# arnavsshah/universal-voice-activity-detection

Hardware: AMD Instinct MI355X
Metric: audio frames/sec (log-mel + PyanNet2 VAD forward); per-frame logit max-abs-err vs CPU ref (higher is better)
Workload: dtype f16x4: f32-equivalent arithmetic on the f16 matrix cores -- exact f32 weights as 3 f16 planes x activations as 2 f16 planes (22 bits), 4 matrix products per f32 product (v_mfma_f32_*_f16; in the recurrence the fourth -- the weights' residue plane, exactly representable as bf8, times h rounded to fp8

## Files before the change

universal-voice-activity-detection_amd/csrc/gemm_f16p_ws.hip:

```cpp
#include "uvad_internal.h"

#include <type_traits>
#include <utility>

namespace uvad {

namespace {

using f32x16 = __attribute__((ext_vector_type(16))) float;
using f16x8 = __attribute__((ext_vector_type(8))) _Float16;
using f32x4 = __attribute__((ext_vector_type(4))) float;
typedef const __attribute__((address_space(1))) void *gptr_t;
typedef __attribute__((address_space(3))) void *lptr_t;

constexpr int SLAB = 128 * 16;
constexpr int STAGE = 2 * SLAB;
constexpr int GROUPS = 8;

template <class F, int... I> __device__ __forceinline__ void static_for_impl(F &&f, std::integer_sequence<int, I...>) {
    (f(std::integral_constant<int, I>{}), ...);
}
template <int N, class F> __device__ __forceinline__ void static_for(F &&f) { static_for_impl(f, std::make_integer_sequence<int, N>{}); }

template <int NKB> struct Ring { static constexpr int NST = NKB % 8 == 0 ? 8 : NKB % 6 == 0 ? 6 : 4; };

template <int N> __device__ __forceinline__ void wait_vm() {
    static_assert(N >= 0 && N <= 63, "vmcnt is a 6-bit counter");
    __builtin_amdgcn_s_waitcnt(0x0f70 | (N & 0xf) | ((N >> 4) << 14));
}

constexpr int NPIECE = 16;
template <int NKB> constexpr int piece_begin(int kb) { return kb >= NKB - 1 ? NPIECE : kb <= 0 ? 0 : (NPIECE * kb) / (NKB - 1); }
template <int NKB> constexpr int stores_in(int from, int to) {
    int n = 0;
    for (int j = from < 1 ? 1 : from; j < to; ++j) n += piece_begin<NKB>(j) - piece_begin<NKB>(j - 1);
    return n;
}

template <int N> __device__ __forceinline__ void wait_vm_lgkm0() {
    static_assert(N >= 0 && N <= 63, "vmcnt is a 6-bit counter");
    __builtin_amdgcn_s_waitcnt(0x0070 | (N & 0xf) | ((N >> 4) << 14));
}

template <int NKB, int NPROD>
__global__ __launch_bounds__(256, 1) void gemm_f16p_ws_kernel(GemmArgs a, int mt, int nt, unsigned *counters) {
    constexpr int NST = Ring<NKB>::NST;
    static_assert(NKB % 2 == 0 && NKB % NST == 0 && NST - 1 <= NKB && NST >= 4, "ring / fragment double-buffer geometry");
    constexpr int SG_LD = 36;
    constexpr int SG_WAVE = 128 * SG_LD * 2;
    __shared__ __attribute__((aligned(16))) unsigned short lds[NST * STAGE + 4 * SG_WAVE + 16];
    int *qword = reinterpret_cast<int *>(lds + NST * STAGE + 4 * SG_WAVE);

    if (a.gate && (*a.gate != 0) != (a.gate_run_if_set != 0)) return;
    const int bid = blockIdx.x, grp = bid & (GROUPS - 1);
    const int n_tile = (bid >> 3) % nt;
    const int tid = threadIdx.x, lane = tid & 63;
    const int wave = __builtin_amdgcn_readfirstlane(tid >> 6);
    const int fr = lane & 31, fh = lane >> 5;

    unsigned *ctr = counters + (size_t)(grp * nt + n_tile) * 32;
    typedef const __attribute__((address_space(4))) int *cint_t;
    cint_t lst = nullptr;
    if (a.ws_tiles) {
        const int d = (a.ws_dirs == 2 && n_tile >= nt / 2) ? 1 : 0;
        lst = (cint_t)(unsigned long long)(a.ws_tiles + a.ws_off[d]);
        mt = a.ws_len[d];
    }
    auto rowtile = [&](int c) { const int i = grp + GROUPS * c; return lst ? lst[i] : i; };
    const int my_tiles = mt > grp ? (mt - grp + GROUPS - 1) / GROUPS : 0;
    if (tid == 0) {
        qword[0] = (int)atomicAdd(ctr, 1u);
        qword[1] = (int)atomicAdd(ctr, 1u);
    }
    __syncthreads();
    int c_cur = __builtin_amdgcn_readfirstlane(qword[0]), c_nxt = __builtin_amdgcn_readfirstlane(qword[1]);
    if ((unsigned)c_cur >= (unsigned)my_tiles) return;
    int r_cur = __builtin_amdgcn_readfirstlane(rowtile(c_cur));
    int r_nxt = (unsigned)c_nxt < (unsigned)my_tiles ? __builtin_amdgcn_readfirstlane(rowtile(c_nxt)) : r_cur;

    static_assert(NPROD == 3 || NPROD == 4, "three or four products");
    f16x8 w0[NKB], w1[NKB], w2[NPROD == 4 ? NKB : 1];
    {
        const size_t wplane = (size_t)((a.N + 127) / 128) * NKB * SLAB;
        const unsigned short *wb = a.Wsplit16 + (size_t)n_tile * NKB * SLAB + (wave * 32 + fr) * 16 + fh * 8;
#pragma unroll
        for (int kb = 0; kb < NKB; ++kb) {
            w0[kb] = *reinterpret_cast<const f16x8 *>(wb + (size_t)kb * SLAB);
            w1[kb] = *reinterpret_cast<const f16x8 *>(wb + wplane + (size_t)kb * SLAB);
            if constexpr (NPROD == 4) w2[kb] = *reinterpret_cast<const f16x8 *>(wb + 2 * wplane + (size_t)kb * SLAB);
        }
    }
    float bias[16];
#pragma unroll
    for (int r = 0; r < 16; ++r) bias[r] = a.bias ? a.bias[n_tile * 128 + wave * 32 + 8 * (r >> 2) + 4 * fh + (r & 3)] : 0.f;
    const float wscale = a.wscale;
    const unsigned q_addr = (unsigned)(size_t)(lptr_t)qword;

    const int ra = tid >> 1;
    const unsigned off = (unsigned)((ra * 2 + ((tid & 1) ^ ((ra >> 3) & 1))) * 8);
    const unsigned short *a_hi = a.Ah + off, *a_lo = a.Al + off;
    auto issue = [&](int stage, int rt, int kb) {
        const size_t t = (size_t)rt * NKB + kb;
        unsigned short *img = lds + stage * STAGE + wave * 512;
        __builtin_amdgcn_global_load_lds((gptr_t)(a_hi + t * SLAB), (lptr_t)(img), 16, 0, 0);
        __builtin_amdgcn_global_load_lds((gptr_t)(a_lo + t * SLAB), (lptr_t)(img + SLAB), 16, 0, 0);
    };

    const unsigned f_base = (unsigned)(size_t)(lptr_t)lds + (unsigned)((fr * 16 + ((fh ^ ((fr >> 3) & 1)) * 8)) * 2);
    f16x8 ah[2][4], al[2][4];
#define UVAD_WS_READ(dst, byte_off) asm volatile("ds_read_b128 %0, %1 offset:%2" : "=v"(dst) : "v"(f_base), "n"(byte_off))
#define UVAD_WS_READ_FRAGS(set, stage)                                                                                       \
    {                                                                                                                      \
        constexpr int base_ = (stage) * (STAGE * 2);                                                                       \
        UVAD_WS_READ(ah[set][0], base_ + 0 * 1024); UVAD_WS_READ(ah[set][1], base_ + 1 * 1024);                            \
        UVAD_WS_READ(ah[set][2], base_ + 2 * 1024); UVAD_WS_READ(ah[set][3], base_ + 3 * 1024);                            \
        UVAD_WS_READ(al[set][0], base_ + SLAB * 2 + 0 * 1024); UVAD_WS_READ(al[set][1], base_ + SLAB * 2 + 1 * 1024);      \
        UVAD_WS_READ(al[set][2], base_ + SLAB * 2 + 2 * 1024); UVAD_WS_READ(al[set][3], base_ + SLAB * 2 + 3 * 1024);      \
    }
    static_assert((NST - 1) * STAGE * 2 + SLAB * 2 + 3 * 1024 < 65536, "DS offset field is 16 bits");

#pragma unroll
    for (int v = 0; v < NST - 1; ++v) issue(v, v < NKB ? r_cur : r_nxt, v % NKB);
    wait_vm<2 * (NST - 2)>();
    __builtin_amdgcn_s_barrier();
    UVAD_WS_READ_FRAGS(0, 0)

    f32x16 hi[4], lo[4];
    const f32x16 zero = {0.f, 0.f, 0.f, 0.f, 0.f, 0.f, 0.f, 0.f, 0.f, 0.f, 0.f, 0.f, 0.f, 0.f, 0.f, 0.f};
    float *sg_w = reinterpret_cast<float *>(lds + NST * STAGE + wave * SG_WAVE) + fr * SG_LD + 4 * fh;
    const unsigned sg_r = (unsigned)(size_t)(lptr_t)(lds + NST * STAGE + wave * SG_WAVE) + (unsigned)(((lane >> 3) * SG_LD + (lane & 7) * 4) * 4);
    const size_t g_lane = (size_t)(lane >> 3) * 64 + (wave & 1) * 32 + (lane & 7) * 4;
    const size_t g_ntile = (size_t)n_tile * 2 + (wave >> 1);
    const int n64 = a.N / 64;
    float *gprev = nullptr;
    f32x4 pc[NPIECE];
#define UVAD_WS_READ_PIECE(p) asm volatile("ds_read_b128 %0, %1 offset:%2" : "=v"(pc[p]) : "v"(sg_r), "n"((p) * 8 * SG_LD * 4))
    static_assert(15 * 8 * SG_LD * 4 < 65536, "DS offset field is 16 bits");
    static_assert(piece_begin<NKB>(1) <= 6 && NPIECE - piece_begin<NKB>(NKB - 2) <= 6, "at most six pieces per k-block (UVAD_WS_PIECES)");

    auto tile = [&](auto first_tag) __attribute__((always_inline)) {
        constexpr bool FIRST = decltype(first_tag)::value;
#pragma unroll
        for (int kb = 0; kb < NKB; ++kb) {
            asm volatile("" : "+a"(w0[kb]), "+a"(w1[kb]));
            if constexpr (NPROD == 4) asm volatile("" : "+a"(w2[kb]));
        }
        float *gout = a.C + ((size_t)r_cur * n64 + g_ntile) * (128 * 64) + g_lane;
        unsigned pulled = 0;
        (void)pc; (void)sg_r;
        static_for<NKB>([&](auto kb_tag) __attribute__((always_inline)) {
            constexpr int kb = decltype(kb_tag)::value;
            constexpr int s = kb & 1, sn = (kb + 1) & 1, stn = (kb + 1) % NST;
            constexpr bool LAST = kb == NKB - 1;
            auto M = [&](auto j_tag) __attribute__((always_inline)) {
                constexpr int j = decltype(j_tag)::value, i = j & 3, p = j >> 2;
                if constexpr (p == 0) hi[i] = __builtin_amdgcn_mfma_f32_32x32x16_f16(w0[kb], ah[s][i], kb == 0 ? zero : hi[i], 0, 0, 0);
                if constexpr (p == 1) lo[i] = __builtin_amdgcn_mfma_f32_32x32x16_f16(w1[kb], ah[s][i], kb == 0 ? zero : lo[i], 0, 0, 0);
                if constexpr (p == 2) lo[i] = __builtin_amdgcn_mfma_f32_32x32x16_f16(w0[kb], al[s][i], lo[i], 0, 0, 0);
                if constexpr (p == 3 && NPROD == 4) lo[i] = __builtin_amdgcn_mfma_f32_32x32x16_f16(w2[kb], ah[s][i], lo[i], 0, 0, 0);
            };
            auto stage_block = [&](int i) __attribute__((always_inline)) {
#pragma unroll
                for (int q = 0; q < 4; ++q) {
                    float4 o;
                    o.x = __builtin_fmaf(__builtin_fmaf(lo[i][4 * q + 0], 0.00048828125f, hi[i][4 * q + 0]), wscale, bias[4 * q + 0]);
                    o.y = __builtin_fmaf(__builtin_fmaf(lo[i][4 * q + 1], 0.00048828125f, hi[i][4 * q + 1]), wscale, bias[4 * q + 1]);
                    o.z = __builtin_fmaf(__builtin_fmaf(lo[i][4 * q + 2], 0.00048828125f, hi[i][4 * q + 2]), wscale, bias[4 * q + 2]);
                    o.w = __builtin_fmaf(__builtin_fmaf(lo[i][4 * q + 3], 0.00048828125f, hi[i][4 * q + 3]), wscale, bias[4 * q + 3]);
                    *reinterpret_cast<float4 *>(sg_w + i * (32 * SG_LD) + 8 * q) = o;
                }
            };
#define UVAD_WS_M(j) M(std::integral_constant<int, (j)>{})
#define UVAD_WS_SB __builtin_amdgcn_sched_barrier(0)
#define UVAD_WS_PIECE_IF(kb_, t_) \
    if constexpr (piece_begin<NKB>(kb_) + (t_) < piece_begin<NKB>((kb_) + 1)) UVAD_WS_READ_PIECE(piece_begin<NKB>(kb_) + (t_));
#define UVAD_WS_STORE_IF(t_)                                                                            \
    if constexpr (piece_begin<NKB>(kb - 1) + (t_) < piece_begin<NKB>(kb))                               \
        __builtin_nontemporal_store(pc[piece_begin<NKB>(kb - 1) + (t_)], reinterpret_cast<f32x4 *>(gprev + (size_t)(piece_begin<NKB>(kb - 1) + (t_)) * (8 * 64)));
            UVAD_WS_SB;
            wait_vm_lgkm0<2 * (NST - 3) + (FIRST ? 0 : stores_in<NKB>(kb - (NST - 3), kb))>();
            __builtin_amdgcn_s_barrier();
            UVAD_WS_SB;
            constexpr int v = kb - 1 + NST;
            const int vr = v < NKB ? r_cur : r_nxt;
            const size_t vt = ((size_t)vr * NKB + v % NKB) * SLAB;
            unsigned short *img = lds + ((kb + NST - 1) % NST) * STAGE + wave * 512;
            constexpr int fb = stn * (STAGE * 2);
#define UVAD_WS_GAP(g)                                                                                                           \
    {                                                                                                                            \
        if constexpr (!FIRST && kb >= 1 && (g) == 0) {                             \
            UVAD_WS_STORE_IF(0) UVAD_WS_STORE_IF(1) UVAD_WS_STORE_IF(2) UVAD_WS_STORE_IF(3) UVAD_WS_STORE_IF(4) UVAD_WS_STORE_IF(5)          \
        }                                                                                                                        \
        if constexpr ((g) == 0) __builtin_amdgcn_global_load_lds((gptr_t)(a_hi + vt), (lptr_t)(img), 16, 0, 0);                   \
        if constexpr ((g) == 1) __builtin_amdgcn_global_load_lds((gptr_t)(a_lo + vt), (lptr_t)(img + SLAB), 16, 0, 0);            \
        if constexpr ((g) == 1) { UVAD_WS_READ(ah[sn][0], fb + 0 * 1024); UVAD_WS_READ(ah[sn][1], fb + 1 * 1024); }              \
        if constexpr ((g) == 2) { UVAD_WS_READ(ah[sn][2], fb + 2 * 1024); UVAD_WS_READ(ah[sn][3], fb + 3 * 1024); }              \
        if constexpr ((g) == 3) { UVAD_WS_READ(al[sn][0], fb + SLAB * 2 + 0 * 1024); UVAD_WS_READ(al[sn][1], fb + SLAB * 2 + 1 * 1024); } \
        if constexpr ((g) == 4) { UVAD_WS_READ(al[sn][2], fb + SLAB * 2 + 2 * 1024); UVAD_WS_READ(al[sn][3], fb + SLAB * 2 + 3 * 1024); } \
        if constexpr ((g) == 5 && !FIRST && !LAST) {                 \
            UVAD_WS_PIECE_IF(kb, 0) UVAD_WS_PIECE_IF(kb, 1) UVAD_WS_PIECE_IF(kb, 2) UVAD_WS_PIECE_IF(kb, 3) UVAD_WS_PIECE_IF(kb, 4) UVAD_WS_PIECE_IF(kb, 5) \
        }                                                                                                                        \
        if constexpr (LAST && (g) == 2) stage_block(0);                                                                          \
        if constexpr (LAST && (g) == 4) stage_block(1);                                                                          \
        if constexpr (LAST && (g) == 6) stage_block(2);                                                                          \
        if constexpr (LAST && (g) == 7) stage_block(3);                                                                          \
        UVAD_WS_SB;                                                                                                              \
    }
            if (kb == 0) {
                unsigned long long sv;
                asm volatile("v_cmp_eq_u32_e32 vcc, 0, %2\n\ts_and_saveexec_b64 %1, vcc\n\tglobal_atomic_add %0, %3, %4, off sc0\n\ts_mov_b64 exec, %1"
                             : "=&v"(pulled), "=&s"(sv) : "v"(tid), "v"(ctr), "v"(1u) : "vcc", "memory");
                UVAD_WS_SB;
            }
            if (kb == NST - 2) {
                unsigned long long sv;
                asm volatile("v_cmp_eq_u32_e32 vcc, 0, %1\n\ts_and_saveexec_b64 %0, vcc\n\tds_write_b32 %2, %3\n\ts_waitcnt lgkmcnt(0)\n\ts_mov_b64 exec, %0"
                             : "=&s"(sv) : "v"(tid), "v"(q_addr), "v"(pulled) : "vcc", "memory");
                UVAD_WS_SB;
            }
            if constexpr (!LAST) {
                UVAD_WS_M(0); UVAD_WS_M(1); UVAD_WS_SB; UVAD_WS_GAP(0)
                UVAD_WS_M(2); UVAD_WS_M(3); UVAD_WS_SB; UVAD_WS_GAP(1)
                UVAD_WS_M(4); UVAD_WS_M(5); UVAD_WS_SB; UVAD_WS_GAP(2)
                UVAD_WS_M(6); UVAD_WS_M(7); UVAD_WS_SB; UVAD_WS_GAP(3)
                UVAD_WS_M(8); UVAD_WS_M(9); UVAD_WS_SB; UVAD_WS_GAP(4)
                UVAD_WS_M(10); UVAD_WS_M(11); UVAD_WS_SB; UVAD_WS_GAP(5)
                UVAD_WS_M(12); UVAD_WS_M(13); UVAD_WS_SB; UVAD_WS_GAP(6)
                UVAD_WS_M(14); UVAD_WS_M(15); UVAD_WS_SB; UVAD_WS_GAP(7)
            } else {
                UVAD_WS_M(0); UVAD_WS_M(4); UVAD_WS_SB; UVAD_WS_GAP(0)
                UVAD_WS_M(8); UVAD_WS_M(12); UVAD_WS_SB; UVAD_WS_GAP(1)
                UVAD_WS_M(1); UVAD_WS_M(5); UVAD_WS_SB; UVAD_WS_GAP(2)
                UVAD_WS_M(9); UVAD_WS_M(13); UVAD_WS_SB; UVAD_WS_GAP(3)
                UVAD_WS_M(2); UVAD_WS_M(6); UVAD_WS_SB; UVAD_WS_GAP(4)
                UVAD_WS_M(10); UVAD_WS_M(14); UVAD_WS_SB; UVAD_WS_GAP(5)
                UVAD_WS_M(3); UVAD_WS_M(7); UVAD_WS_SB; UVAD_WS_GAP(6)
                UVAD_WS_M(11); UVAD_WS_M(15); UVAD_WS_SB; UVAD_WS_GAP(7)
            }
        });
        int c_nn;
        asm volatile("ds_read_b32 %0, %1\n\ts_waitcnt lgkmcnt(0)" : "=v"(c_nn) : "v"(q_addr) : "memory");
        gprev = gout;
        c_cur = c_nxt;
        r_cur = r_nxt;
        c_nxt = __builtin_amdgcn_readfirstlane(c_nn);
        r_nxt = (unsigned)c_nxt < (unsigned)my_tiles ? __builtin_amdgcn_readfirstlane(rowtile(c_nxt)) : r_cur;
    };
    tile(std::true_type{});
    for (int done = 1; done < my_tiles && (unsigned)c_cur < (unsigned)my_tiles; ++done) tile(std::false_type{});
    static_for<NPIECE>([&](auto t) __attribute__((always_inline)) {
        constexpr int p = decltype(t)::value;
        f32x4 o;
        asm volatile("ds_read_b128 %0, %1 offset:%2\n\ts_waitcnt lgkmcnt(0)" : "=v"(o) : "v"(sg_r), "n"(p * 8 * SG_LD * 4) : "memory");
        __builtin_nontemporal_store(o, reinterpret_cast<f32x4 *>(gprev + (size_t)p * (8 * 64)));
    });
    wait_vm<0>();
}

}

size_t gemm_f16p_ws_counter_bytes() { return (size_t)GROUPS * 8 * 32 * sizeof(unsigned); }

bool gemm_f16p_ws_supported(const GemmArgs &a, int n_cu) {
    if (a.out_planes || !a.c_blocked || a.act != 0 || a.N % 128 != 0 || a.N / 128 > 8) return false;
    if (a.K != 64 && a.K != 96 && a.K != 128 && a.K != 256) return false;
    const long mt = (a.M + 127) / 128;
    return mt * (a.N / 128) >= 2L * (n_cu > 0 ? n_cu : 256);
}

hipError_t launch_gemm_f16p_ws(const GemmArgs &a, unsigned *counters, int n_cu, hipStream_t s) {
    if (!gemm_f16p_ws_supported(a, n_cu) || !counters || !a.Ah || !a.Al || !a.Wsplit16 || !a.C || a.ldw != a.K) return hipErrorInvalidValue;
    const int mt = (a.M + 127) / 128, nt = a.N / 128;
    if (a.ws_tiles) {
        if ((a.ws_dirs != 1 && a.ws_dirs != 2) || (a.ws_dirs == 2 && nt % 2 != 0)) return hipErrorInvalidValue;
        for (int d = 0; d < a.ws_dirs; ++d)
            if (a.ws_off[d] < 0 || a.ws_len[d] < 0 || a.ws_len[d] > mt) return hipErrorInvalidValue;
    }
    hipError_t e = launch_zero_counters(counters, (int)(gemm_f16p_ws_counter_bytes() / sizeof(unsigned)), s);
    if (e != hipSuccess) return e;
    const int per = GROUPS * nt;
    int grid = (n_cu > 0 ? n_cu : 256) / per * per;
    if (grid < per) grid = per;
    if (a.products != 0 && a.products != 3 && a.products != 4) return hipErrorInvalidValue;
    const bool three = a.products == 3;
#define UVAD_WS_LAUNCH(NKB_)                                                                                                          \
    if (three) hipLaunchKernelGGL((gemm_f16p_ws_kernel<NKB_, 3>), dim3(grid), dim3(256), 0, s, a, mt, nt, counters);                   \
    else hipLaunchKernelGGL((gemm_f16p_ws_kernel<NKB_, 4>), dim3(grid), dim3(256), 0, s, a, mt, nt, counters);
    switch (a.K / 16) {
        case 4: UVAD_WS_LAUNCH(4) break;
        case 6: UVAD_WS_LAUNCH(6) break;
        case 8: UVAD_WS_LAUNCH(8) break;
        case 16: UVAD_WS_LAUNCH(16) break;
        default: return hipErrorInvalidValue;
    }
#undef UVAD_WS_LAUNCH
    return hipGetLastError();
}

}
```

universal-voice-activity-detection_amd/csrc/uvad_internal.h:

```cpp
#pragma once
#include <hip/hip_runtime.h>
#include <type_traits>
#include <stdint.h>

namespace uvad {

constexpr int SEQ_TILE = 4;

constexpr int PLANE_TILE = 128;
__host__ __device__ inline size_t plane_index(size_t row, int col, int width) {
    return ((row / PLANE_TILE) * (size_t)(width / 16) + (size_t)(col / 16)) * (PLANE_TILE * 16) + (row % PLANE_TILE) * 16 + (size_t)(col % 16);
}
inline size_t plane_rows(size_t M) { return (M + PLANE_TILE - 1) / PLANE_TILE * PLANE_TILE; }

__host__ __device__ inline size_t g_index(size_t row, int col, int ncols) {
    return ((row / 128) * (size_t)(ncols / 64) + (size_t)(col / 64)) * (128 * 64) + (row % 128) * 64 + (size_t)(col % 64);
}

struct GemmArgs {
    const float *A;
    const float *W;
    const unsigned short *Ah, *Al;
    const unsigned short *Wsplit16;
    float wscale;
    unsigned short *Ch, *Cl;
    int out_planes;
    int products;
    int c_blocked;
    int ldw;
    const float *bias;
    float *C;
    int M, N, K;
    int lda, ldc;
    int a_mode, B, T;
    float leaky_slope;
    int act;
    const int *gate;
    int gate_run_if_set;
    const int *ws_tiles;
    int ws_off[2], ws_len[2], ws_dirs;
};
hipError_t launch_gemm(const GemmArgs &a, hipStream_t s);
int gemm_padded_k(int K);
hipError_t launch_gemm_f16p(const GemmArgs &a, hipStream_t s);
int gemm_f16p_padded_k(int K);
bool gemm_f16p_ws_supported(const GemmArgs &a, int n_cu);
size_t gemm_f16p_ws_counter_bytes();
hipError_t launch_gemm_f16p_ws(const GemmArgs &a, unsigned *counters, int n_cu, hipStream_t s);
size_t weight_plane_elems(int N, int ldw);
bool split_weights_f16x3(const float *w, int N, int ldw, unsigned short *out , float *wscale);
hipError_t launch_mask_features(const float *x, int B, int T, int F, const int *lens, float *out, hipStream_t s);
hipError_t launch_split_features(const float *x, int B, int T, int F, int Fp, int tiles, unsigned short *xh, unsigned short *xl, int *flag,
                                 hipStream_t s);

struct LstmArgs {
    const float *G; int ldg;
    const float *Whh_packed;
    const unsigned *Whh16h_regs; const unsigned short *Whh16h_p2; const float *whh16h_scale;
    const unsigned short *Whh16h_p2q; int p2q_scale;
    float *Y; int ldy;
    unsigned short *Yh, *Yl;
    int products;
    int tiles, T, H, dirs;
    int steps, t_begin[2];
    int tile_mode;
    int n_cu;
    const float *h0, *c0; float *hN, *cN;
    const int *lens; int nB;
};
hipError_t launch_lstm(const LstmArgs &a, hipStream_t s, int *tile_used = nullptr);
int lstm_auto_tile(int tiles, int dirs, int H, int n_cu);
size_t whh_packed_elems(int H);
int lstm_waves(int H);
void pack_whh(const float *w_hh, int H, float *out);
size_t whh16h_regs_elems();
size_t whh16h_p2_elems();
bool pack_whh16h(const float *w_hh, unsigned *regs, unsigned short *p2, float *wscale);
size_t whh16h_p2q_elems();
bool pack_whh16h_p2q(const float *w_hh, unsigned short *p2q, int *scale);

struct ClsArgs {
    const float *Z; int ldz, K;
    const float *w, *b;
    float *logits, *probs;
    int tiles, T, B;
    int ld_out;
};
hipError_t launch_classifier(const ClsArgs &a, hipStream_t s);
hipError_t launch_untile(const void *src, const void *src_lo, int lds_, int W, float *dst, int tiles, int T, int B, hipStream_t s);
hipError_t launch_median(const float *probs, int B, int T, int kernel, uint8_t *labels, hipStream_t s);
hipError_t launch_runs(const uint8_t *labels, int B, int T, int max_runs, int *runs, int *counts, hipStream_t s);
hipError_t launch_lens_fill(float *logits, float *probs, int B, int T, int ld, const int *lens, hipStream_t s);
hipError_t launch_median_lens(const float *probs, int B, int T, int kernel, uint8_t *labels, const int *lens, hipStream_t s);
hipError_t launch_runs_lens(const uint8_t *labels, int B, int T, int max_runs, int *runs, int *counts, const int *lens, hipStream_t s);
hipError_t launch_der(const uint8_t *pred, const uint8_t *gt, int B, int T, uint32_t *counts, hipStream_t s);

hipError_t launch_zero_counters(unsigned *p, int n, hipStream_t s);

hipError_t launch_spin(unsigned long long ticks, unsigned long long *sink, hipStream_t s);

struct HeadArgs {
    const unsigned short *Yh, *Yl;
    long long M; int K1;
    const unsigned short *W1, *W2;
    float w1scale, w2scale;
    const float *b1, *b2, *wc, *bc;
    float slope;
    float *logits, *probs;
    int tiles, T, B, ld_out;
    unsigned *counter;
    int products;
};
bool head_fused_supported(int K1, int lin_hidden, int lin_layers, long long M, int n_cu);
hipError_t launch_head_fused(const HeadArgs &a, int n_cu, hipStream_t s);

struct FbankTables {
    const float *window;
    const int *mel_start;
    const int *mel_len;
    const float *mel_w;
    const float *mel_wt;
    int mel_stride;
    const float *tw512;
    int nyquist;
};
__host__ __device__ inline int mel_image_ld(int n_mels) { return n_mels <= 64 ? 64 : 128; }
__host__ __device__ inline size_t mel_image_floats(int mel_stride, int n_mels) { return (size_t)mel_stride * mel_image_ld(n_mels); }
struct FbankArgs {
    const void *pcm; int pcm_is_i16;
    int B; int64_t S; int64_t T;
    int64_t row_stride;
    int frame_len, frame_shift, n_mels;
    float preemph, log_floor; int remove_dc, snip_edges;
    float *feats;
    unsigned short *plane_hi, *plane_lo; int plane_w;
    const float *vs_chunk, *vs_tail_in; float *vs_tail_out;
    int vs_tail, vs_chunk_len, vs_first, vs_n_left, vs_offset;
    FbankTables tab;
    const int64_t *nsamp;
};
hipError_t launch_fbank(const FbankArgs &a, hipStream_t s);
hipError_t launch_frames_of(const int64_t *nsamp, int B, int64_t S, int frame_len, int frame_shift, int snip_edges, int *frames, hipStream_t s);
size_t fbank_lds_bytes(const FbankArgs &a);
hipError_t launch_stream_stage(const float *chunk_pcm, int B, int chunk, int tail, int n_left, int first_step,
                               const float *tail_in, float *tail_out, float *staging, hipStream_t s);

struct WindowArgs {
    const float *newf; float *ring; const long long *ctr_in; long long *ctr_out;
    int B, R, F, k, Tw;
    int planes; unsigned short *xh, *xl; int Fp, tiles;
    float *out;
};
hipError_t launch_window_assemble(const WindowArgs &a, hipStream_t s);
hipError_t launch_window_carry(const long long *ctr_in, long long *ctr_out, hipStream_t s);
hipError_t launch_window_emit(const float *logits_in, const float *probs_in, int B, int Tw, int r0, int n, float *logits, float *probs,
                              int ld_out, hipStream_t s);

struct WavWindowArgs {
    const void *chunk; void *ring; const long long *ctr_in; long long *ctr_out;
    int B, chunk_len, J, R, Tw, Sw;
    long long ring_len;
    void *out;
};
hipError_t launch_wav_window_assemble(const WavWindowArgs &a, int is_i16, hipStream_t s);

struct SlotCounters { long long *n, *e; int *active, *tw_last; long long *step; };
struct alignas(16) SlotPlan {
    long long n, e, e_prev;
    int live, end, first, k;
    int offset, Tw, r0, n_emit;
    int pad[2];
};
struct SlotStageArgs {
    const float *chunk; const uint8_t *flags; SlotCounters ctr;
    float *tails;
    float *staging; SlotPlan *plan;
    int B, chunk_len, frame_len, shift, n_left, row, W, L;
};
hipError_t launch_slot_stage(const SlotStageArgs &a, hipStream_t s);
struct SlotAssembleArgs {
    const SlotPlan *plan; SlotCounters ctr;
    const float *newf; int kmax; float *ring;
    int B, W, F;
    int planes; unsigned short *xh, *xl; int Fp, tiles;
    float *out; int *lens;
};
hipError_t launch_slot_assemble(const SlotAssembleArgs &a, hipStream_t s);
struct WavSlotArgs {
    const void *chunk; const uint8_t *flags; SlotCounters ctr;
    void *ring; long long ring_len;
    void *out; int Sw_max; long long *nsamp; SlotPlan *plan;
    int B, chunk_len, J, R, W, L;
};
hipError_t launch_wav_slot_assemble(const WavSlotArgs &a, int is_i16, hipStream_t s);
struct SlotEmitArgs {
    const SlotPlan *plan; SlotCounters ctr;
    const float *logits_in, *probs_in; int B, W;
    float *logits, *probs; int ld_out; int *counts;
};
hipError_t launch_slot_emit(const SlotEmitArgs &a, hipStream_t s);

struct SlidingPlan {
    const int *first; int nrec; long long N; int W, Hf;
    const int *lens; int T;
    const long long *nsamp; long long S; int J, R0;
};
struct SlidingAssembleArgs {
    SlidingPlan plan; const float *feats; long long i0; int Bg, F;
    int planes; unsigned short *xh, *xl; int Fp, tiles;
    float *out; int *lens; int *flag;
};
hipError_t launch_sliding_assemble(const SlidingAssembleArgs &a, hipStream_t s);
struct SlidingWavArgs {
    SlidingPlan plan; const void *pcm; long long i0; int Bg; long long Sw;
    void *out; long long *nsamp_out;
};
hipError_t launch_sliding_wav_gather(const SlidingWavArgs &a, int is_i16, hipStream_t s);
struct SlidingAggregateArgs {
    SlidingPlan plan; const float *win, *weights;
    float *out; int ld_out; int *frames;
};
hipError_t launch_sliding_aggregate(const SlidingAggregateArgs &a, hipStream_t s);

constexpr int LSTM_STACK_TMAX = 4, LSTM_STACK_MAX_LAYERS = 8, LSTM_STACK_MAX_LIN = 4;
struct LstmStackArgs {
    const float *feats; int kin0;
    const float *wih[LSTM_STACK_MAX_LAYERS];
    const float *whh[LSTM_STACK_MAX_LAYERS];
    const float *bias[LSTM_STACK_MAX_LAYERS];
    int n_layers;
    float *h, *c; size_t layer_stride;
    float *Y; int ldy;
    unsigned short *Yh, *Yl;
    int tiles, T, B;
    const float *lin_w[LSTM_STACK_MAX_LIN], *lin_b[LSTM_STACK_MAX_LIN]; int n_lin;
    const float *cls_w, *cls_b; float slope;
    float *logits, *probs; int ld_out;
    FbankArgs fb; int fb_on;
};
size_t lstm_stack_fb_lds_bytes(const FbankArgs &fb, int T);
bool lstm_stack_supported(int hidden, int dirs, int in_dim, int T, int n_layers);
hipError_t launch_lstm_stack(const LstmStackArgs &a, hipStream_t s);
size_t lstm_image_elems(int K);
void pack_lstm_image(const float *w , int K, float *out);
size_t fc_image_elems();
void pack_fc_image(const float *w , float *out);

struct SincRows { const int *lin, *lpool, *prefix; };
struct SincNoRows {};
template <class A> struct SincLensArgs : A { SincRows rows; };
template <bool LENS, class A> using SincArgsT = typename std::conditional<LENS, SincLensArgs<A>, A>::type;
template <bool LENS> using SincRowsArg = typename std::conditional<LENS, SincRows, SincNoRows>::type;
template <bool LENS> using SincRowTArg = typename std::conditional<LENS, const int *, SincNoRows>::type;
struct SincRowCursor { int b, tile, end, lin, lpool; };
__device__ __forceinline__ void sinc_cursor_at(const SincRows &r, int b, long long g, SincRowCursor &c) {
    c.b = b; c.tile = (int)(g - r.prefix[b]); c.end = r.prefix[b + 1]; c.lin = r.lin[b]; c.lpool = r.lpool[b];
}
__device__ __forceinline__ SincRowCursor sinc_cursor_seek(const SincRows &r, int B, long long g) {
    int lo = 0, hi = B;
    while (hi - lo > 1) {
        const int mid = (lo + hi) >> 1;
        if (r.prefix[mid] <= g) lo = mid; else hi = mid;
    }
    SincRowCursor c;
    sinc_cursor_at(r, lo, g, c);
    return c;
}
__device__ __forceinline__ void sinc_cursor_next(const SincRows &r, long long g, SincRowCursor &c) {
    if (g < c.end) { ++c.tile; return; }
    int b = c.b + 1;
    while (r.prefix[b + 1] <= g) ++b;
    sinc_cursor_at(r, b, g, c);
}

struct SincConvArgs {
    const float *in; long long in_bstride; int Cin, Lin;
    const int16_t *in_i16;
    const float *in_scale, *in_shift;
    int in_lrelu; float slope;
    const float *Wt2;
    const float *bias;
    int Kw, stride, Ktot, Kp, Cout, do_abs;
    int Lconv, Lpool, ntiles;
    float *out;
    float *partials;
    int B;
    int n_cu;
};
hipError_t launch_wav_stats(const float *wav, int B, long long S, long long row_stride, const float *gamma, const float *beta, float eps,
                            float *scale, float *shift, hipStream_t s, const int *row_n = nullptr);
hipError_t launch_wav_stats(const int16_t *wav, int B, long long S, long long row_stride, const float *gamma, const float *beta, float eps,
                            float *scale, float *shift, hipStream_t s, const int *row_n = nullptr);
struct SincConvPlan { int waves, pt, phases; };
SincConvPlan sinc_conv_plan(const SincConvArgs &a);
hipError_t launch_sinc_conv(const SincConvArgs &a, hipStream_t s, const SincRows *rows = nullptr);
size_t sinc_conv_lds_bytes(const SincConvArgs &a, int NT, int waves);
int sinc_conv_ept(const SincConvArgs &a, int waves);
hipError_t launch_norm_finalize(const float *partials, int B, int ntiles, int pt, int phases, int NW, int C, int L, const float *gamma,
                                const float *beta, float eps, float *scale, float *shift, hipStream_t s, const SincRows *rows = nullptr);
hipError_t launch_sinc_out(const float *P, const float *scale, const float *shift, int B, int C, int L, float slope, float *feats, int ldf,
                           hipStream_t s, const int *row_T = nullptr);

constexpr int SINC_GEO_ARRAYS = 19;
struct SincGeoArgs {
    const int64_t *nsamp; int B; long long S;
    int kw[3], stride0, pt[3];
    int *geo;
};
hipError_t launch_sinc_row_geometry(const SincGeoArgs &g, hipStream_t s);

struct SincF16Args {
    const float *in; long long in_bstride; int Lin;
    const int16_t *in_i16;
    const float *in_scale, *in_shift; int n_in;
    float slope;
    const unsigned short *Wfrag; float wscale;
    const float *bias;
    int Lpool, ntiles;
    float *out;
    float *partials;
    int B, n_cu;
};
bool sinc_f16p_supported(int n_filters, int kernel_size, int stride, int c2, int k2, int c3, int k3);
int sinc_f16p_ksteps(int stage);
int sinc_f16p_cst(int stage);
int sinc_f16p_ntiles(long long Lpool);
size_t sinc_f16p_partial_floats(int stage, int B, int ntiles);
size_t sinc_f16p_wfrag_elems(int stage);
bool sinc_f16p_pack_weights(int stage, const float *w, int nrows, int ldk, unsigned short *out, float *wscale);
hipError_t launch_sinc_conv_f16p(int stage, const SincF16Args &a, hipStream_t s, const SincRows *rows = nullptr);
hipError_t launch_norm_finalize_f16p(int stage, const float *partials, int B, int ntiles, int C, int L, const float *gamma, const float *beta, float eps,
                                     float *scale, float *shift, hipStream_t s, const SincRows *rows = nullptr);
hipError_t launch_sinc_out_f16p(const float *P, const float *scale, const float *shift, int B, int C, int CST, int L, float slope, float *feats, int ldf,
                                hipStream_t s, const int *row_T = nullptr);

constexpr int INGEST_MAX_PHASES = 8, INGEST_MAX_TAPS = 64, INGEST_MAX_CHANNELS = 8;
struct IngestArgs {
    const void *in; int enc, C; long long S_in;
    const long long *nsamp;
    const float *taps; int up, down, width, K;
    float *out; long long S_out;
    long long *out_nsamp;
    float *hist; long long *seen; const uint8_t *flags; int H, Dj;
    int B;
};
hipError_t launch_ingest(const IngestArgs &a, hipStream_t s);

constexpr int EP_HIST_WORDS = 4;
constexpr unsigned EP_MAGIC = 0x55564550u;
// ... 169 lines not shown
```

Before: 62.54 million.

## Add paired-wave K-split work-stealing GEMM kernel for K=128/256 four-product path

Result: slower. 53.94 million (-13.7%).

```diff
diff --git a/universal-voice-activity-detection_amd/csrc/gemm_f16p_ws.hip b/universal-voice-activity-detection_amd/csrc/gemm_f16p_ws.hip
--- a/universal-voice-activity-detection_amd/csrc/gemm_f16p_ws.hip
+++ b/universal-voice-activity-detection_amd/csrc/gemm_f16p_ws.hip
@@ -257,6 +257,318 @@
     wait_vm<0>();
 }
 
+constexpr int PT = 64;
+constexpr int PUNIT = 2 * PT * 16;
+constexpr int PSTAGE = 2 * PUNIT;
+constexpr int PNST = 4;
+constexpr int PNPIECE = 8;
+template <int H> constexpr int pp_begin(int p) { return p >= H - 1 ? PNPIECE : p <= 0 ? 0 : (PNPIECE * p) / (H - 1); }
+
+template <int NKB, int NPROD>
+__global__ __launch_bounds__(512, 1) void gemm_f16p_ws_pair_kernel(GemmArgs a, int mt, int nt, unsigned *counters) {
+    constexpr int H = NKB / 2;
+    static_assert(NKB % 2 == 0 && H % PNST == 0 && PNST == 4, "the stage of a step is a constant; the vmcnt counts below are for four stages");
+    static_assert(NPROD == 3 || NPROD == 4, "three or four products");
+    constexpr int SG_LD = 36;
+    constexpr int SG_WAVE = PT * SG_LD * 2;
+    constexpr int HO_PAIR = 64 * 64 * 2;
+    constexpr int HO0 = PNST * PSTAGE, SG0 = HO0 + 4 * HO_PAIR, Q0 = SG0 + 4 * SG_WAVE;
+    static_assert((Q0 + 16) * 2 <= 160 * 1024, "LDS budget");
+    __shared__ __attribute__((aligned(16))) unsigned short lds[Q0 + 16];
+    int *qword = reinterpret_cast<int *>(lds + Q0);
+
+    if (a.gate && (*a.gate != 0) != (a.gate_run_if_set != 0)) return;
+    const int bid = blockIdx.x, grp = bid & (GROUPS - 1);
+    const int n_tile = (bid >> 3) % nt;
+    const int tid = threadIdx.x, lane = tid & 63;
+    const int wave = __builtin_amdgcn_readfirstlane(tid >> 6);
+    const int cw = wave & 3;
+    const bool stage_b = wave >= 4;
+    const int fr = lane & 31, fh = lane >> 5;
+
+    unsigned *ctr = counters + (size_t)(grp * nt + n_tile) * 32;
+    typedef const __attribute__((address_space(4))) int *cint_t;
+    cint_t lst = nullptr;
+    if (a.ws_tiles) {
+        const int d = (a.ws_dirs == 2 && n_tile >= nt / 2) ? 1 : 0;
+        lst = (cint_t)(unsigned long long)(a.ws_tiles + a.ws_off[d]);
+        mt = a.ws_len[d];
+    }
+    auto rowtile = [&](int c) { const int i = grp + GROUPS * c; return lst ? lst[i] : i; };
+    const int my_tiles = mt > grp ? (mt - grp + GROUPS - 1) / GROUPS : 0;
+    if (tid == 0) {
+        qword[0] = (int)atomicAdd(ctr, 1u);
+        qword[1] = (int)atomicAdd(ctr, 1u);
+    }
+    __syncthreads();
+    int c_cur = __builtin_amdgcn_readfirstlane(qword[0]), c_nxt = __builtin_amdgcn_readfirstlane(qword[1]);
+    if ((unsigned)c_cur >= (unsigned)my_tiles) return;
+    int r_cur = __builtin_amdgcn_readfirstlane(rowtile(c_cur));
+    int r_nxt = (unsigned)c_nxt < (unsigned)my_tiles ? __builtin_amdgcn_readfirstlane(rowtile(c_nxt)) : r_cur;
+    int r_prev = r_cur, half = 0, done = 1;
+    bool a_valid = true;
+    const unsigned q_addr = (unsigned)(size_t)(lptr_t)qword;
+    auto advance = [&]() __attribute__((always_inline)) {
+        if (!a_valid) return false;
+        if (half) {
+            int c_nn;
+            asm volatile("ds_read_b32 %0, %1\n\ts_waitcnt lgkmcnt(0)" : "=v"(c_nn) : "v"(q_addr) : "memory");
+            r_prev = r_cur;
+            c_cur = c_nxt;
+            r_cur = r_nxt;
+            c_nxt = __builtin_amdgcn_readfirstlane(c_nn);
+            r_nxt = (unsigned)c_nxt < (unsigned)my_tiles ? __builtin_amdgcn_readfirstlane(rowtile(c_nxt)) : r_cur;
+            a_valid = done < my_tiles && (unsigned)c_cur < (unsigned)my_tiles;
+            ++done;
+        }
+        half ^= 1;
+        return true;
+    };
+
+    f16x8 w0[H], w1[H], w2[NPROD == 4 ? H : 1];
+    {
+        const int kb0 = stage_b ? H : 0;
+        const size_t wplane = (size_t)((a.N + 127) / 128) * NKB * SLAB;
+        const unsigned short *wb = a.Wsplit16 + ((size_t)n_tile * NKB + kb0) * SLAB + (cw * 32 + fr) * 16 + fh * 8;
+#pragma unroll
+        for (int k4 = 0; k4 < H; k4 += 4) {
+#pragma unroll
+            for (int kb = k4; kb < k4 + 4; ++kb) {
+                w0[kb] = *reinterpret_cast<const f16x8 *>(wb + (size_t)kb * SLAB);
+                w1[kb] = *reinterpret_cast<const f16x8 *>(wb + wplane + (size_t)kb * SLAB);
+                if constexpr (NPROD == 4) w2[kb] = *reinterpret_cast<const f16x8 *>(wb + 2 * wplane + (size_t)kb * SLAB);
+            }
+#pragma unroll
+            for (int kb = k4; kb < k4 + 4; ++kb) {
+                asm volatile("" : "+a"(w0[kb]), "+a"(w1[kb]));
+                if constexpr (NPROD == 4) asm volatile("" : "+a"(w2[kb]));
+            }
+        }
+    }
+    const unsigned f_base = (unsigned)(size_t)(lptr_t)lds + (stage_b ? PUNIT * 2 : 0) + (unsigned)((fr * 16 + ((fh ^ ((fr >> 3) & 1)) * 8)) * 2);
+    f16x8 ah[2][2], al[2][2];
+#define UVAD_WP_READ(dst, byte_off) asm volatile("ds_read_b128 %0, %1 offset:%2" : "=a"(dst) : "v"(f_base), "n"(byte_off))
+    f32x16 hi[2], lo[2];
+    const f32x16 zero = {0.f, 0.f, 0.f, 0.f, 0.f, 0.f, 0.f, 0.f, 0.f, 0.f, 0.f, 0.f, 0.f, 0.f, 0.f, 0.f};
+    static_assert((PNST - 1) * PSTAGE * 2 + PUNIT * 2 + 3 * 1024 < 65536, "DS offset field is 16 bits");
+#define UVAD_WP_READ_FRAGS(set, stage)                                                                                   \
+    {                                                                                                                    \
+        constexpr int base_ = (stage) * (PSTAGE * 2);                                                                    \
+        UVAD_WP_READ(ah[set][0], base_ + 0 * 1024); UVAD_WP_READ(ah[set][1], base_ + 1 * 1024);                          \
+        UVAD_WP_READ(al[set][0], base_ + 2 * 1024); UVAD_WP_READ(al[set][1], base_ + 3 * 1024);                          \
+    }
+#define UVAD_WP_M(P, j, Z)                                                                                                        \
+    {                                                                                                                            \
+        constexpr int i_ = (j) & 1, pr_ = (j) >> 1, s_ = (P) & 1;                                                                \
+        if constexpr (pr_ == 0) hi[i_] = __builtin_amdgcn_mfma_f32_32x32x16_f16(w0[P], ah[s_][i_], (Z) ? zero : hi[i_], 0, 0, 0); \
+        if constexpr (pr_ == 1) lo[i_] = __builtin_amdgcn_mfma_f32_32x32x16_f16(w1[P], ah[s_][i_], (Z) ? zero : lo[i_], 0, 0, 0); \
+        if constexpr (pr_ == 2) lo[i_] = __builtin_amdgcn_mfma_f32_32x32x16_f16(w0[P], al[s_][i_], lo[i_], 0, 0, 0);              \
+        if constexpr (pr_ == 3 && NPROD == 4) lo[i_] = __builtin_amdgcn_mfma_f32_32x32x16_f16(w2[P], ah[s_][i_], lo[i_], 0, 0, 0); \
+    }
+#define UVAD_WP_PIN_W                                                        \
+    _Pragma("unroll") for (int kb = 0; kb < H; ++kb) {                       \
+        asm volatile("" : "+a"(w0[kb]), "+a"(w1[kb]));                       \
+        if constexpr (NPROD == 4) asm volatile("" : "+a"(w2[kb]));           \
+    }
+    float *ho = reinterpret_cast<float *>(lds + HO0 + cw * HO_PAIR) + lane * 4;
+
+    if (!stage_b) {
+        const int ra = (cw & 1) * 32 + (lane >> 1);
+        const unsigned short *a_src = (cw >> 1 ? a.Al : a.Ah) + (unsigned)((ra * 2 + ((lane & 1) ^ ((ra >> 3) & 1))) * 8);
+        auto src_off = [&](int rt, int hf, int kb) { return ((size_t)rt * NKB + kb) * SLAB + (size_t)hf * (PT * 16); };
+#pragma unroll
+        for (int v = 0; v < PNST - 1; ++v) {
+            unsigned short *img = lds + v * PSTAGE + cw * 512;
+            __builtin_amdgcn_global_load_lds((gptr_t)(a_src + src_off(r_cur, 0, v)), (lptr_t)(img), 16, 0, 0);
+            __builtin_amdgcn_global_load_lds((gptr_t)(a_src + src_off(r_cur, 0, H + v)), (lptr_t)(img + PUNIT), 16, 0, 0);
+        }
+        wait_vm<2 * (PNST - 2)>();
+        __builtin_amdgcn_s_barrier();
+        UVAD_WP_READ_FRAGS(0, 0)
+        unsigned pulled = 0;
+        for (;;) {
+            const int rp = half ? r_cur : r_prev, rn = half ? r_nxt : r_cur, hx = half ^ 1;
+            (void)f_base; (void)ah; (void)al; (void)q_addr; (void)ctr; (void)tid; (void)pulled;
+            static_for<H>([&](auto p_tag) __attribute__((always_inline)) {
+                constexpr int p = decltype(p_tag)::value;
+                constexpr int sn = (p + 1) & 1, stn = (p + 1) % PNST;
+                constexpr bool LAST = p == H - 1;
+                (void)f_base; (void)ah; (void)al; (void)q_addr; (void)ctr; (void)tid; (void)pulled;
+                UVAD_WS_SB;
+                wait_vm_lgkm0<2 * (PNST - 3)>();
+                __builtin_amdgcn_s_barrier();
+                UVAD_WS_SB;
+                constexpr int q = p + PNST - 1, kq = q % H;
+                const size_t ta = q < H ? src_off(r_cur, half, kq) : src_off(rn, hx, kq);
+                const size_t tb = q < H ? src_off(rp, hx, H + kq) : src_off(r_cur, half, H + kq);
+                unsigned short *img = lds + (q % PNST) * PSTAGE + cw * 512;
+                constexpr int fb = stn * (PSTAGE * 2);
+                if constexpr (p == 0) {
+                    if (half == 0) {
+                        unsigned long long sv;
+                        asm volatile("v_cmp_eq_u32_e32 vcc, 0, %2\n\ts_and_saveexec_b64 %1, vcc\n\tglobal_atomic_add %0, %3, %4, off sc0\n\ts_mov_b64 exec, %1"
+                                     : "=&v"(pulled), "=&s"(sv) : "v"(tid), "v"(ctr), "v"(1u) : "vcc", "memory");
+                    }
+                    UVAD_WS_SB;
+                }
+                if constexpr (p == H - 2) {
+                    if (half == 1) {
+                        unsigned long long sv;
+                        asm volatile("v_cmp_eq_u32_e32 vcc, 0, %1\n\ts_and_saveexec_b64 %0, vcc\n\tds_write_b32 %2, %3\n\ts_waitcnt lgkmcnt(0)\n\ts_mov_b64 exec, %0"
+                                     : "=&s"(sv) : "v"(tid), "v"(q_addr), "v"(pulled) : "vcc", "memory");
+                    }
+                    UVAD_WS_SB;
+                }
+                auto hand = [&](int i) __attribute__((always_inline)) {
+#pragma unroll
+                    for (int qd = 0; qd < 4; ++qd) {
+                        f32x4 h = {hi[i][4 * qd], hi[i][4 * qd + 1], hi[i][4 * qd + 2], hi[i][4 * qd + 3]};
+                        f32x4 l = {lo[i][4 * qd], lo[i][4 * qd + 1], lo[i][4 * qd + 2], lo[i][4 * qd + 3]};
+                        *reinterpret_cast<f32x4 *>(ho + (i * 8 + qd) * 256) = h;
+                        *reinterpret_cast<f32x4 *>(ho + (i * 8 + 4 + qd) * 256) = l;
+                    }
+                };
+#define UVAD_WP_A_GAP(g)                                                                                                       \
+    {                                                                                                                          \
+        if constexpr ((g) == 0) __builtin_amdgcn_global_load_lds((gptr_t)(a_src + ta), (lptr_t)(img), 16, 0, 0);              \
+        if constexpr ((g) == 1) __builtin_amdgcn_global_load_lds((gptr_t)(a_src + tb), (lptr_t)(img + PUNIT), 16, 0, 0);      \
+        if constexpr ((g) == 1) { UVAD_WP_READ(ah[sn][0], fb + 0 * 1024); UVAD_WP_READ(ah[sn][1], fb + 1 * 1024); }            \
+        if constexpr ((g) == 2) { UVAD_WP_READ(al[sn][0], fb + 2 * 1024); UVAD_WP_READ(al[sn][1], fb + 3 * 1024); }            \
+        if constexpr (LAST && (g) == 2) hand(0);                                                                               \
+        if constexpr (LAST && (g) == 3) hand(1);                                                                               \
+        UVAD_WS_SB;                                                                                                            \
+    }
+                if constexpr (!LAST) {
+                    UVAD_WP_M(p, 0, p == 0) UVAD_WP_M(p, 1, p == 0) UVAD_WS_SB; UVAD_WP_A_GAP(0)
+                    UVAD_WP_M(p, 2, p == 0) UVAD_WP_M(p, 3, p == 0) UVAD_WS_SB; UVAD_WP_A_GAP(1)
+                    UVAD_WP_M(p, 4, false) UVAD_WP_M(p, 5, false) UVAD_WS_SB; UVAD_WP_A_GAP(2)
+                    UVAD_WP_M(p, 6, false) UVAD_WP_M(p, 7, false) UVAD_WS_SB; UVAD_WP_A_GAP(3)
+                } else {
+                    UVAD_WP_M(p, 0, false) UVAD_WP_M(p, 2, false) UVAD_WS_SB; UVAD_WP_A_GAP(0)
+                    UVAD_WP_M(p, 4, false) UVAD_WP_M(p, 6, false) UVAD_WS_SB; UVAD_WP_A_GAP(1)
+                    UVAD_WP_M(p, 1, false) UVAD_WP_M(p, 3, false) UVAD_WS_SB; UVAD_WP_A_GAP(2)
+                    UVAD_WP_M(p, 5, false) UVAD_WP_M(p, 7, false) UVAD_WS_SB; UVAD_WP_A_GAP(3)
+                }
+            });
+            UVAD_WS_SB;
+            wait_vm_lgkm0<63>();
+            UVAD_WS_SB;
+            if (!advance()) break;
+        }
+        wait_vm<0>();
+    } else {
+        float bias[16];
+#pragma unroll
+        for (int r = 0; r < 16; ++r) bias[r] = a.bias ? a.bias[n_tile * 128 + cw * 32 + 8 * (r >> 2) + 4 * fh + (r & 3)] : 0.f;
+        const float wscale = a.wscale;
+        float *sg_w = reinterpret_cast<float *>(lds + SG0 + cw * SG_WAVE) + fr * SG_LD + 4 * fh;
+        const unsigned sg_r = (unsigned)(size_t)(lptr_t)(lds + SG0 + cw * SG_WAVE) + (unsigned)(((lane >> 3) * SG_LD + (lane & 7) * 4) * 4);
+        const size_t g_lane = (size_t)(lane >> 3) * 64 + (cw & 1) * 32 + (lane & 7) * 4;
+        const size_t g_ntile = (size_t)n_tile * 2 + (cw >> 1);
+        const int n64 = a.N / 64;
+        float *gprev = nullptr;
+        f32x4 pc[PNPIECE];
+#define UVAD_WP_READ_PIECE(p_) asm volatile("ds_read_b128 %0, %1 offset:%2" : "=v"(pc[p_]) : "v"(sg_r), "n"((p_) * 8 * SG_LD * 4))
+        static_assert(pp_begin<H>(1) <= 3 && PNPIECE - pp_begin<H>(H - 2) <= 3, "at most three pieces per step");
+        __builtin_amdgcn_s_barrier();
+
+        auto round = [&](auto first_tag) __attribute__((always_inline)) {
+            constexpr bool FIRST = decltype(first_tag)::value;
+            (void)f_base; (void)ah; (void)al; (void)pc; (void)sg_r;
+            static_for<H>([&](auto p_tag) __attribute__((always_inline)) {
+                constexpr int p = decltype(p_tag)::value;
+                constexpr int sn = (p + 1) & 1, stn = (p + 1) % PNST;
+                constexpr bool LAST = p == H - 1;
+                constexpr int fb = stn * (PSTAGE * 2);
+                (void)f_base; (void)ah; (void)al; (void)pc; (void)sg_r;
+                UVAD_WS_SB;
+                wait_vm_lgkm0<63>();
+                __builtin_amdgcn_s_barrier();
+                UVAD_WS_SB;
+                if constexpr (p == 0) {
+#pragma unroll
+                    for (int i = 0; i < 2; ++i) {
+                        const f32x4 h0 = *reinterpret_cast<const f32x4 *>(ho + (i * 8 + 0) * 256), h1 = *reinterpret_cast<const f32x4 *>(ho + (i * 8 + 1) * 256);
+                        const f32x4 h2 = *reinterpret_cast<const f32x4 *>(ho + (i * 8 + 2) * 256), h3 = *reinterpret_cast<const f32x4 *>(ho + (i * 8 + 3) * 256);
+                        const f32x4 l0 = *reinterpret_cast<const f32x4 *>(ho + (i * 8 + 4) * 256), l1 = *reinterpret_cast<const f32x4 *>(ho + (i * 8 + 5) * 256);
+                        const f32x4 l2 = *reinterpret_cast<const f32x4 *>(ho + (i * 8 + 6) * 256), l3 = *reinterpret_cast<const f32x4 *>(ho + (i * 8 + 7) * 256);
+                        hi[i] = __builtin_shufflevector(__builtin_shufflevector(h0, h1, 0, 1, 2, 3, 4, 5, 6, 7), __builtin_shufflevector(h2, h3, 0, 1, 2, 3, 4, 5, 6, 7),
+                                                        0, 1, 2, 3, 4, 5, 6, 7, 8, 9, 10, 11, 12, 13, 14, 15);
+                        lo[i] = __builtin_shufflevector(__builtin_shufflevector(l0, l1, 0, 1, 2, 3, 4, 5, 6, 7), __builtin_shufflevector(l2, l3, 0, 1, 2, 3, 4, 5, 6, 7),
+                                                        0, 1, 2, 3, 4, 5, 6, 7, 8, 9, 10, 11, 12, 13, 14, 15);
+                    }
+                    UVAD_WS_SB;
+                }
+                auto stage_block = [&](int i) __attribute__((always_inline)) {
+#pragma unroll
+                    for (int qd = 0; qd < 4; ++qd) {
+                        float4 o;
+                        o.x = __builtin_fmaf(__builtin_fmaf(lo[i][4 * qd + 0], 0.00048828125f, hi[i][4 * qd + 0]), wscale, bias[4 * qd + 0]);
+                        o.y = __builtin_fmaf(__builtin_fmaf(lo[i][4 * qd + 1], 0.00048828125f, hi[i][4 * qd + 1]), wscale, bias[4 * qd + 1]);
+                        o.z = __builtin_fmaf(__builtin_fmaf(lo[i][4 * qd + 2], 0.00048828125f, hi[i][4 * qd + 2]), wscale, bias[4 * qd + 2]);
+                        o.w = __builtin_fmaf(__builtin_fmaf(lo[i][4 * qd + 3], 0.00048828125f, hi[i][4 * qd + 3]), wscale, bias[4 * qd + 3]);
+                        *reinterpret_cast<float4 *>(sg_w + i * (32 * SG_LD) + 8 * qd) = o;
+                    }
+                };
+#define UVAD_WP_PIECE_IF(t_) \
+    if constexpr (pp_begin<H>(p) + (t_) < pp_begin<H>(p + 1)) UVAD_WP_READ_PIECE(pp_begin<H>(p) + (t_));
+#define UVAD_WP_STORE_IF(t_)                                                                        \
+    if constexpr (pp_begin<H>(p - 1) + (t_) < pp_begin<H>(p))                                       \
+        __builtin_nontemporal_store(pc[pp_begin<H>(p - 1) + (t_)], reinterpret_cast<f32x4 *>(gprev + (size_t)(pp_begin<H>(p - 1) + (t_)) * (8 * 64)));
+#define UVAD_WP_B_GAP(g)                                                                                                       \
+    {                                                                                                                          \
+        if constexpr (!FIRST && p >= 1 && (g) == 0) { UVAD_WP_STORE_IF(0) UVAD_WP_STORE_IF(1) UVAD_WP_STORE_IF(2) }              \
+        if constexpr ((g) == 1) { UVAD_WP_READ(ah[sn][0], fb + 0 * 1024); UVAD_WP_READ(ah[sn][1], fb + 1 * 1024); }            \
+        if constexpr ((g) == 2) { UVAD_WP_READ(al[sn][0], fb + 2 * 1024); UVAD_WP_READ(al[sn][1], fb + 3 * 1024); }            \
+        if constexpr (!FIRST && !LAST && (g) == 3) { UVAD_WP_PIECE_IF(0) UVAD_WP_PIECE_IF(1) UVAD_WP_PIECE_IF(2) }              \
+        if constexpr (LAST && (g) == 2) stage_block(0);                                                                        \
+        if constexpr (LAST && (g) == 3) stage_block(1);                                                                        \
+        UVAD_WS_SB;                                                                                                            \
+    }
+                if constexpr (!LAST) {
+                    UVAD_WP_M(p, 0, false) UVAD_WP_M(p, 1, false) UVAD_WS_SB; UVAD_WP_B_GAP(0)
+                    UVAD_WP_M(p, 2, false) UVAD_WP_M(p, 3, false) UVAD_WS_SB; UVAD_WP_B_GAP(1)
+                    UVAD_WP_M(p, 4, false) UVAD_WP_M(p, 5, false) UVAD_WS_SB; UVAD_WP_B_GAP(2)
+                    UVAD_WP_M(p, 6, false) UVAD_WP_M(p, 7, false) UVAD_WS_SB; UVAD_WP_B_GAP(3)
+                } else {
+                    UVAD_WP_M(p, 0, false) UVAD_WP_M(p, 2, false) UVAD_WS_SB; UVAD_WP_B_GAP(0)
+                    UVAD_WP_M(p, 4, false) UVAD_WP_M(p, 6, false) UVAD_WS_SB; UVAD_WP_B_GAP(1)
+                    UVAD_WP_M(p, 1, false) UVAD_WP_M(p, 3, false) UVAD_WS_SB; UVAD_WP_B_GAP(2)
+                    UVAD_WP_M(p, 5, false) UVAD_WP_M(p, 7, false) UVAD_WS_SB; UVAD_WP_B_GAP(3)
+                }
+            });
+        };
+        for (int rnd = 0;; rnd = rnd < 2 ? rnd + 1 : 2) {
+            const int rp = half ? r_cur : r_prev, hx = half ^ 1;
+            float *gout = a.C + ((size_t)rp * n64 + g_ntile) * (128 * 64) + (size_t)hx * (PT * 64) + g_lane;
+            if (rnd == 0) {
+#pragma unroll
+                for (int p = 0; p < H; ++p) {
+                    UVAD_WS_SB;
+                    __builtin_amdgcn_s_barrier();
+                    UVAD_WS_SB;
+                }
+                UVAD_WP_READ_FRAGS(0, 0)
+            } else {
+                if (rnd == 1) round(std::true_type{});
+                else round(std::false_type{});
+                gprev = gout;
+            }
+            UVAD_WS_SB;
+            wait_vm_lgkm0<63>();
+            UVAD_WS_SB;
+            if (!advance()) break;
+        }
+        static_for<PNPIECE>([&](auto t) __attribute__((always_inline)) {
+            constexpr int p = decltype(t)::value;
+            (void)sg_r;
+            f32x4 o;
+            asm volatile("ds_read_b128 %0, %1 offset:%2\n\ts_waitcnt lgkmcnt(0)" : "=v"(o) : "v"(sg_r), "n"(p * 8 * SG_LD * 4) : "memory");
+            __builtin_nontemporal_store(o, reinterpret_cast<f32x4 *>(gprev + (size_t)p * (8 * 64)));
+        });
+    }
+}
+
 }
 
 size_t gemm_f16p_ws_counter_bytes() { return (size_t)GROUPS * 8 * 32 * sizeof(unsigned); }
@@ -266,6 +578,10 @@
     if (a.K != 64 && a.K != 96 && a.K != 128 && a.K != 256) return false;
     const long mt = (a.M + 127) / 128;
     return mt * (a.N / 128) >= 2L * (n_cu > 0 ? n_cu : 256);
+}
+
+bool gemm_f16p_ws_paired(const GemmArgs &a, int n_cu) {
+    return gemm_f16p_ws_supported(a, n_cu) && (a.K == 128 || a.K == 256) && a.products != 3;
 }
 
 hipError_t launch_gemm_f16p_ws(const GemmArgs &a, unsigned *counters, int n_cu, hipStream_t s) {
@@ -283,6 +599,11 @@
     if (grid < per) grid = per;
     if (a.products != 0 && a.products != 3 && a.products != 4) return hipErrorInvalidValue;
     const bool three = a.products == 3;
+    if (gemm_f16p_ws_paired(a, n_cu)) {
+        if (a.K == 256) hipLaunchKernelGGL((gemm_f16p_ws_pair_kernel<16, 4>), dim3(grid), dim3(512), 0, s, a, mt, nt, counters);
+        else hipLaunchKernelGGL((gemm_f16p_ws_pair_kernel<8, 4>), dim3(grid), dim3(512), 0, s, a, mt, nt, counters);
+        return hipGetLastError();
+    }
 #define UVAD_WS_LAUNCH(NKB_)                                                                                                          \
     if (three) hipLaunchKernelGGL((gemm_f16p_ws_kernel<NKB_, 3>), dim3(grid), dim3(256), 0, s, a, mt, nt, counters);                   \
     else hipLaunchKernelGGL((gemm_f16p_ws_kernel<NKB_, 4>), dim3(grid), dim3(256), 0, s, a, mt, nt, counters);
diff --git a/universal-voice-activity-detection_amd/csrc/uvad_internal.h b/universal-voice-activity-detection_amd/csrc/uvad_internal.h
--- a/universal-voice-activity-detection_amd/csrc/uvad_internal.h
+++ b/universal-voice-activity-detection_amd/csrc/uvad_internal.h
@@ -45,6 +45,7 @@
 hipError_t launch_gemm_f16p(const GemmArgs &a, hipStream_t s);
 int gemm_f16p_padded_k(int K);
 bool gemm_f16p_ws_supported(const GemmArgs &a, int n_cu);
+bool gemm_f16p_ws_paired(const GemmArgs &a, int n_cu);
 size_t gemm_f16p_ws_counter_bytes();
 hipError_t launch_gemm_f16p_ws(const GemmArgs &a, unsigned *counters, int n_cu, hipStream_t s);
 size_t weight_plane_elems(int N, int ldw);
```
